# brdav/refign

Measured on AMD Instinct MI355X. Metric: image-pairs/s (align+seg fwd+bwd, 1080x1920), higher is better.
Workload: dtype bf16

## Files before the change

### include/refign_hip.h

```cpp
#ifndef REFIGN_HIP_H
#define REFIGN_HIP_H

#ifdef __cplusplus
extern "C" {
#endif

#define RFN_OK 0
#define RFN_EINVAL (-1)
#define RFN_ELAUNCH (-2)
#define RFN_ENOTSUP (-3)
#define RFN_ENONDET (-4)

#define RFN_ABI_VERSION 5

typedef void* rfn_stream_t;

int rfn_abi_version(void);
const char* rfn_last_error(void);

int rfn_set_deterministic(int on);
int rfn_get_deterministic(void);

int rfn_corr_fwd_f32(const float* in1, const float* in2, float* out, int B, int C, int iH, int iW,
                     int kH, int kW, int patchH, int patchW, int padH, int padW, int dilH, int dilW,
// ... 96 lines not shown

unsigned long rfn_sum_rows_workspace_bytes(long S, long n);
int rfn_sum_rows(const void* x, float* out, void* workspace, long S, long n, int x_dtype, int accumulate,
                 rfn_stream_t stream);
int rfn_linear_param_grads(const void* grad_y, float* grad_bias, void* workspace, long T, long N, int acc_bias,
                           const void* w_partials, float* grad_weight, int S, long NK, int acc_weight, int dtype,
                           rfn_stream_t stream);

int rfn_multi_cast_chunk_elems(void);
int rfn_multi_permute_chunk_elems(void);
int rfn_multi_permute_cast_f32(const void* table, int nchunks, rfn_stream_t stream);
int rfn_multi_cast_f32_bf16(const void* table, int nchunks, rfn_stream_t stream);
int rfn_multi_cast_f32_f16(const void* table, int nchunks, rfn_stream_t stream);
int rfn_multi_ema_f32(const void* table, int nchunks, float momentum, rfn_stream_t stream);
int rfn_multi_transpose_cast_f32_bf16(const void* table, int ntiles, rfn_stream_t stream);
int rfn_multi_transpose_cast_f32_f16(const void* table, int ntiles, rfn_stream_t stream);
int rfn_multi_transpose_tile(void);
int rfn_multi_adamw_f32(const void* table, int nchunks, const float* group_args, int ngroups, rfn_stream_t stream);
int rfn_amp_unscale_f32(float* grads, long n, const float* scale, float* found_inf, rfn_stream_t stream);
int rfn_multi_adamw_amp_f32(const void* table, int nchunks, const double* group_args, int ngroups, const float* found_inf,
                            const float* step, rfn_stream_t stream);
int rfn_amp_update_scale(float* scale, int* growth_tracker, const float* found_inf, float* step, float growth_factor,
                         float backoff_factor, int growth_interval, rfn_stream_t stream);

int rfn_upsample_concat_nhwc(const void* src0, const void* src1, const void* src2, const void* src3, const int* hs,
                             const int* ws, const int* cs, int nlev, void* out, int n, int H, int W, int dtype,
                             rfn_stream_t stream);
int rfn_upsample_concat_nhwc_bwd(const void* grad_out, void* grad0, void* grad1, void* grad2, void* grad3, const int* hs,
                                 const int* ws, const int* cs, int nlev, int n, int H, int W, int dtype,
                                 rfn_stream_t stream);

int rfn_patchify_tokens(const void* src, void* dst, int B, int H, int W, int C, int r, int dtype, int inverse,
                        rfn_stream_t stream);

int rfn_patchify_tokens_cmajor(const void* src, void* dst, int B, int H, int W, int C, int r, int dtype, int inverse,
                               rfn_stream_t stream);

int rfn_gemm_nt(const void* X, const void* W, const void* bias, const void* res, const float* rowscale,
                int rows_per_sample, int act, void* Y, long M, long N, long K, long ldx, long ldw, long ldy, int dtype,
                rfn_stream_t stream);
int rfn_conv2d_nhwc(const void* X, const void* W, const void* bias, const void* res, int act, void* Y, int B, int H,
                    int Wd, int C, int N, int KH, int KW, int stride, int pad, int dil, long ldw, long ldy, int dtype,
                    rfn_stream_t stream);
int rfn_gemm_tn(const void* G, const void* X, float* P, long T, long N, long K, long ldg, long ldx, int rows_per_slab,
                int accumulate, float* grad_bias, const float* rowscale, int rows_per_sample, int dtype,
                rfn_stream_t stream);
int rfn_gemm_tn_grouped(int count, const void* const* G, const void* const* X, float* const* P, float* const* grad_bias,
                        const float* const* rowscale, const long* T, const long* N, const long* K, const long* ldg,
                        const long* ldx, const int* rows_per_slab, const int* rows_per_sample, int dtype, rfn_stream_t stream);

int rfn_attn_pack(const void* src, long batch_stride, long row_stride, int B, int heads, int nrows, int nblk, void* rpack,
                  void* tpack, const void* src2, void* rpack2, void* tpack2, rfn_stream_t stream);
int rfn_attn_fwd(const void* Q, long q_batch_stride, long q_row_stride, const void* k_rpack, const void* v_tpack, void* O,
                 long o_batch_stride, long o_row_stride, float* lse2, int B, int heads, int Nq, int Nkv, int nkblk,
                 int nqpad, float scale, int kv_pack_heads, int dtype, rfn_stream_t stream);
int rfn_attn_bwd_dq(const void* Q, long q_batch_stride, long q_row_stride, const void* dO, const void* O,
                    long o_batch_stride, long o_row_stride, const void* k_rpack, const void* v_rpack, const void* k_tpack,
                    const float* lse2, float* delta, void* dQ, long dq_batch_stride, long dq_row_stride, int B, int heads,
                    int Nq, int Nkv, int nkblk, int nqpad, float scale, int kv_pack_heads, int dtype,
                    rfn_stream_t stream);
int rfn_attn_bwd_dkv(const void* K, const void* V, long kv_batch_stride, long kv_row_stride, const void* q_rpack,
                     const void* q_tpack, const void* do_rpack, const void* do_tpack, const float* lse2,
                     const float* delta, float* accT, void* dKV, int B, int heads, int Nq, int Nkv, int nqblk, int nqpad,
                     int nkpad, int blocks_per_chunk, float scale, int dtype, rfn_stream_t stream);

int rfn_attn32_fwd(const float* Q, long q_batch_stride, long q_row_stride, const float* KV, long kv_batch_stride,
                   long kv_row_stride, float* O, long o_batch_stride, long o_row_stride, float* lse2, int B, int heads,
                   int head_dim, int Nq, int Nkv, int nqpad, float scale, rfn_stream_t stream);
int rfn_attn32_bwd(const float* Q, long q_batch_stride, long q_row_stride, const float* KV, long kv_batch_stride,
                   long kv_row_stride, const float* dO, const float* O, long o_batch_stride, long o_row_stride,
                   const float* lse2, float* delta, float* dQ, long dq_batch_stride, long dq_row_stride, float* dKV,
                   long dkv_batch_stride, long dkv_row_stride, int B, int heads, int head_dim, int Nq, int Nkv, int nqpad,
                   int query_chunks, float scale, rfn_stream_t stream);

int rfn_split3_bf16(const float* x, long x_row_stride, void* out, long out_row_stride, long term_stride, long rows, int K,
                    int Kp, int order, rfn_stream_t stream);
int rfn_split3_cat_bf16(const float* const* parts, const long* strides, const int* channels, int nparts, void* out, int B, int H,
                        int W, int Cp, rfn_stream_t stream);

int rfn_ffn_fc1_dw_gelu_bf16(const void* x, const void* w1, const void* b1, const float* wdw_tap, const float* bdw, void* a,
                             int views, int H, int W, int C, int HID, rfn_stream_t stream);
int rfn_ffn_fc1_dw_gelu_f16(const void* x, const void* w1, const void* b1, const float* wdw_tap, const float* bdw, void* a,
                            int views, int H, int W, int C, int HID, rfn_stream_t stream);

int rfn_bn_stats_fwd(const void* x, double* sums, long T, int C, int dtype, rfn_stream_t stream);
int rfn_bn_apply_fwd(const void* x, const float* gamma, const float* beta, void* y, const double* sums, float* running_mean,
                     float* running_var, long T, int C, float eps, float momentum, int relu, int dtype, rfn_stream_t stream);
int rfn_bn_apply_fwd_ld(const void* x, const float* gamma, const float* beta, void* y, long ld_y, const double* sums,
                        float* running_mean, float* running_var, long T, int C, float eps, float momentum, int relu, int dtype,
                        rfn_stream_t stream);
int rfn_bn_stats_bwd(const void* x, const void* grad_y, const double* fwd_sums, const float* gamma, const float* beta,
                     float* bwd_sums, long T, int C, float eps, int relu, int dtype, rfn_stream_t stream);
int rfn_bn_apply_bwd(const void* x, const void* grad_y, const double* fwd_sums, const float* bwd_sums, const float* gamma,
                     const float* beta, void* grad_x, long T, int C, float eps, int relu, int dtype, rfn_stream_t stream);
int rfn_bn_train_fwd(const void* x, const float* gamma, const float* beta, void* y, double* sums, float* running_mean,
                     float* running_var, long T, int C, float eps, float momentum, int relu, int dtype,
                     rfn_stream_t stream);
int rfn_bn_train_bwd(const void* x, const void* grad_y, const double* fwd_sums, const float* gamma, const float* beta,
                     void* grad_x, float* bwd_sums, long T, int C, float eps, int relu, int dtype, rfn_stream_t stream);

int rfn_upsample_ce(const void* logits, const long* target, const float* weight, float* grad_lo, double* loss_sum, int B,
                    int C, int h, int w, int H, int W, int ignore_index, int dtype, int round16, rfn_stream_t stream);

int rfn_slide_argmax_confmat(const void* crop_logits, int dtype, int B, int C, int h, int w, const int* boxes, int nbox, int H,
                             int W, const long* target, int ignore_index, unsigned char* labels, long* confmat,
                             rfn_stream_t stream);

int rfn_gemm_nt_o32(const void* X, const void* W, const float* bias, const float* res, const float* rowscale,
                    int rows_per_sample, int act, float* Y, long M, long N, long K, long ldx, long ldw, long ldy,
                    rfn_stream_t stream);
int rfn_conv2d_nhwc_o32(const void* X, const void* W, const float* bias, int act, float* Y, int B, int H, int Wd, int C, int N,
                        int KH, int KW, int stride, int pad, int dil, long ldw, long ldy, int transposed,
                        rfn_stream_t stream);
int rfn_conv2d_nhwc_dgrad(const void* GY, const void* Wt, void* DX, int B, int H, int W, int C, int N, int KH, int KW,
                          int stride, int pad, int dil, long ldw, long ldy, int dtype, rfn_stream_t stream);
int rfn_conv2d_nhwc_wgrad(const void* GY, const void* X, float* P, float* grad_bias, int B, int H, int W, int C, int N, int KH,
                          int KW, int stride, int pad, int dil, long ldg, long Kpad, int rows_per_slab, int accumulate,
                          int dtype, rfn_stream_t stream);

int rfn_dacs_mix_jitter(const float* src, const float* trg, const long* gt_src, const long* pseudo_label,
                        const float* pseudo_weight, float* mixed_img, long* mixed_lbl, float* mixed_weight, double* mean_ws,
                        int B, int H, int W, const long* class_bits, const int* jitter_on, const int* order,
                        const float* factor, const float* hue, const float* mean3, const float* std3,
                        rfn_stream_t stream);
int rfn_dacs_blur(const float* x, float* tmp, float* y, int B, int C, int H, int W, int ksize_y, int ksize_x, const int* blur_on,
                  const double* sigma_y, const double* sigma_x, rfn_stream_t stream);

int rfn_crop_label_hist_u8(const void* label, int H, int W, const int* boxes, int K, int* hist, rfn_stream_t stream);
int rfn_crop_flip_norm_u8(const void* image, const void* label, int C, int H, int W, int top, int left, int h, int w, int flip,
                          const float* mean3, const float* std3, float* out_image, long* out_label, rfn_stream_t stream);

int rfn_resize_crop_flip_norm_u8(const void* image_hwc, int H, int W, int Hd, int Wd, const int* bounds_x, const int* coef_x, int kmax_x,
                                 const int* bounds_y, const int* coef_y, int kmax_y, int top, int left, int h, int w, int flip,
                                 const float* mean3, const float* std3, float* out_image, rfn_stream_t stream);
int rfn_resize_u8(const void* image_hwc, int H, int W, int Hd, int Wd, const int* bounds_x, const int* coef_x, int kmax_x,
                  const int* bounds_y, const int* coef_y, int kmax_y, void* out_chw, rfn_stream_t stream);
int rfn_resize_nearest_u8(const void* label, int H, int W, int Hd, int Wd, const int* ytab, const int* xtab, void* out,
                          rfn_stream_t stream);

int rfn_resize_filter_u8(const void* image_hwc, int H, int W, int Hd, int Wd, int filter, const int* bounds_x, const int* coef_x,
                         int kmax_x, const int* bounds_y, const int* coef_y, int kmax_y, void* out_chw, rfn_stream_t stream);
int rfn_resize_filter_crop_flip_norm_pad_u8(const void* image_hwc, int H, int W, int Hd, int Wd, int filter, const int* bounds_x,
                                            const int* coef_x, int kmax_x, const int* bounds_y, const int* coef_y, int kmax_y, int top,
                                            int left, int h, int w, int flip, const float* mean3, const float* std3, float* out_image,
                                            int Hf, int Wf, rfn_stream_t stream);

int rfn_sparse_epe_f32(const float* flow, const float* conf, const float* pts_src, const float* pts_trg, const int* offsets, int B,
                       int h, int w, double* rows, rfn_stream_t stream);

int rfn_gemm_nt_f8(const void* X8, const void* W8, const float* wscale, float x_scale, const void* bias, const void* res,
                   const float* rowscale, int rows_per_sample, int act, void* Y, int out_f8, float out_q, long M, long N,
                   long K, long ldx, long ldw, long ldy, rfn_stream_t stream);
int rfn_quant_rows_f8(const void* table, int nchunks, rfn_stream_t stream);
int rfn_quant_f8(const void* x_bf16, void* y8, long n, float q, rfn_stream_t stream);
int rfn_layernorm_fwd_f8(const void* x_bf16, const float* gamma, const float* beta, void* y8, long rows, int C, float eps,
                         float out_q, rfn_stream_t stream);
int rfn_dwconv3x3_gelu_nhwc_fwd_f8(const void* x8, const float* weight, const float* bias, void* y8, int B, int H, int W, int C,
                                   float x_scale, float out_q, rfn_stream_t stream);
int rfn_attn_pack_f8(const void* kv8, long batch_stride, long row_stride, int B, int heads, int Nkv, int nst, void* pack,
                     rfn_stream_t stream);
int rfn_attn_fwd_f8(const void* q8, long q_batch_stride, long q_row_stride, const void* pack, void* o8, long o_batch_stride,
                    long o_row_stride, int B, int heads, int Nq, int Nkv, int nst, float scale, float q_scale, float k_scale,
                    float v_scale, float out_q, rfn_stream_t stream);

unsigned long rfn_bn_stats_det_workspace_bytes(long T, int C);
int rfn_bn_stats_fwd_det(const void* x, double* sums, void* workspace, long T, int C, int dtype, rfn_stream_t stream);
// ... 77 lines not shown
```

### refign_amd/mfma.py

```python
import ctypes
import os

import torch

from . import _lib, determinism
from ._tensor import ptr
from ._tensor import DTYPE_CODE16 as _DT16

ENABLED = True

LIBRARY_CALLS = {}
_NOTE = True


def note_library(kind, *tensors):
    if not _NOTE or not tensors or not tensors[0].is_cuda:
        return
    key = (kind, str(tensors[0].dtype).replace("torch.", ""), tuple(tuple(t.shape) for t in tensors))
    n = LIBRARY_CALLS.get(key)
    if n is None and len(LIBRARY_CALLS) < 4096:
        if os.environ.get("RFN_LOG_LIBRARY", "0") == "1":
            print(f"[refign_amd] library fallback: {kind} {key[1]} {key[2]}", flush=True)
        LIBRARY_CALLS[key] = 1
    elif n is not None:
# ... 222 lines not shown
            X = arr(vp, [t[1].data_ptr() for t in grp])
            P = arr(vp, [t[2].data_ptr() for t in grp])
            Bv = arr(vp, [None if t[3] is None else t[3].data_ptr() for t in grp])
            R = arr(vp, [None if t[4] is None else t[4].data_ptr() for t in grp])
            T = arr(lg, [t[0].shape[0] for t in grp])
            N = arr(lg, [t[0].shape[1] for t in grp])
            K = arr(lg, [t[1].shape[1] for t in grp])
            ldg = arr(lg, [t[0].stride(0) for t in grp])
            ldx = arr(lg, [t[1].stride(0) for t in grp])
            rps = arr(it_, [t[6] for t in grp])
            rsa = arr(it_, [t[5] for t in grp])
            cast = lambda a_: ctypes.cast(a_, vp)
            _lib.call("rfn_gemm_tn_grouped", dev, n, cast(G), cast(X), cast(P), cast(Bv), cast(R), cast(T), cast(N), cast(K),
                      cast(ldg), cast(ldx), cast(rps), cast(rsa), _DT16[dt])


class deferred_wgrads:

    def __enter__(self):
        global _WGRAD_QUEUE
        self._outer = _WGRAD_QUEUE
        if GROUP_WGRADS and ENABLED and self._outer is None:
            _WGRAD_QUEUE = []
        return self

    def __exit__(self, *exc):
        global _WGRAD_QUEUE
        if self._outer is None and _WGRAD_QUEUE is not None:
            try:
                if exc[0] is None:
                    flush_wgrads()
            finally:
                _WGRAD_QUEUE = None
        return False


class _WgradMark(torch.autograd.Function):

    @staticmethod
    def forward(ctx, x):
        return x.view_as(x)

    @staticmethod
    def backward(ctx, g):
        flush_wgrads()
        return g


def wgrad_mark(x):
    return _WgradMark.apply(x) if (GROUP_WGRADS and torch.is_grad_enabled() and x.requires_grad) else x


_PACK_BLOCK = 4096


def _pack(src, batch_stride, row_stride, B, heads, nrows, nblk, want_r=True, want_t=True, src2=None):
    dev = src.device
    nbytes = B * heads * nblk * _PACK_BLOCK
    new = lambda want: torch.empty(nbytes, dtype=torch.uint8, device=dev) if want else None
    r, t = new(want_r), new(want_t)
    r2, t2 = (new(want_r), new(want_t)) if src2 is not None else (None, None)
    _lib.call("rfn_attn_pack", dev, ptr(src), batch_stride, row_stride, B, heads, nrows, nblk, ptr(r), ptr(t), ptr(src2),
              ptr(r2), ptr(t2))
    return (r, t), (r2, t2)


def _attn_ok(q, kv, heads):
    if not (ENABLED and q.is_cuda and q.dtype in _DT16 and kv.dtype == q.dtype and q.dim() == 3 and kv.dim() == 3):
        return False
    B, N, C = q.shape
    return (C == heads * 64 and kv.shape[0] == B and kv.shape[2] == 2 * C and q.is_contiguous() and kv.is_contiguous()
            and q.data_ptr() % 16 == 0 and kv.data_ptr() % 16 == 0)


def _dims(q, kv):
    B, N, C = q.shape
    Nkv = kv.shape[1]
    nkblk = -(-Nkv // 32)
    nkblk += nkblk & 1
    nqblk = -(-N // 32)
    return B, N, C, Nkv, nkblk, nqblk, nqblk * 32


def _fwd(q, kv, heads, scale, need_bwd):
    B, N, C, Nkv, nkblk, nqblk, nqpad = _dims(q, kv)
    dev = q.device
    (kvr, kvt), _ = _pack(kv, kv.stride(0), kv.stride(1), B, 2 * heads, Nkv, nkblk)
    voff = heads * nkblk * _PACK_BLOCK
    o = torch.empty_like(q)
    lse2 = torch.empty((B * heads, nqpad), dtype=torch.float32, device=dev)
    _lib.call("rfn_attn_fwd", dev, ptr(q), q.stride(0), q.stride(1), kvr.data_ptr(), kvt.data_ptr() + voff, ptr(o), o.stride(0),
              o.stride(1), ptr(lse2), B, heads, N, Nkv, nkblk, nqpad, float(scale), 2 * heads, _DT16[q.dtype])
    return o, lse2, (kvr, kvt)


def _chunk_blocks(nqblk, Nkv, BH):
    kblocks = -(-Nkv // 256)
    chunks = max(1, 128 // max(1, kblocks * BH))
    return max(4, -(-nqblk // chunks))


class _AttnFn(torch.autograd.Function):
    @staticmethod
    def forward(ctx, q, kv, heads, scale):
        need = q.requires_grad or kv.requires_grad
        o, lse2, packs = _fwd(q, kv, heads, scale, need)
        if need:
            ctx.save_for_backward(q, kv, o, lse2, *packs)
            ctx.heads, ctx.scale = heads, scale
        return o

    @staticmethod
    def backward(ctx, do):
        q, kv, o, lse2, kvr, kvt = ctx.saved_tensors
        heads, scale = ctx.heads, ctx.scale
        B, N, C, Nkv, nkblk, nqblk, nqpad = _dims(q, kv)
        dev = q.device
        if do.dtype != q.dtype:
            do = do.to(q.dtype)
        if not do.is_contiguous():
            do = do.contiguous()
        dt = _DT16[q.dtype]
        dq = torch.empty_like(q)
        delta = torch.empty_like(lse2)
        voff = heads * nkblk * _PACK_BLOCK
        _lib.call("rfn_attn_bwd_dq", dev, ptr(q), q.stride(0), q.stride(1), ptr(do), ptr(o), o.stride(0), o.stride(1),
                  kvr.data_ptr(), kvr.data_ptr() + voff, kvt.data_ptr(), ptr(lse2), ptr(delta), ptr(dq), dq.stride(0),
                  dq.stride(1), B, heads, N, Nkv, nkblk, nqpad, float(scale), 2 * heads, dt)
        (qr, qt), (gr, gt) = _pack(q, q.stride(0), q.stride(1), B, heads, N, nqblk, src2=do)
        nkpad = -(-Nkv // 32) * 32
        chunk = _chunk_blocks(nqblk, Nkv, B * heads)
        det = determinism.enabled()
        images = -(-nqblk // chunk) if det else 1
        accT = torch.empty(images * B * heads * 2 * 64 * nkpad, dtype=torch.float32, device=dev)
        dkv = torch.empty_like(kv)
        k_view, v_view = kv[:, :, :C], kv[:, :, C:]
        _lib.call("rfn_attn_bwd_dkv_det" if det else "rfn_attn_bwd_dkv", dev, ptr(k_view), ptr(v_view), kv.stride(0), kv.stride(1),
                  ptr(qr), ptr(qt), ptr(gr), ptr(gt), ptr(lse2), ptr(delta), ptr(accT), ptr(dkv), B, heads, N, Nkv, nqblk, nqpad,
                  nkpad, chunk, float(scale), dt)
        return dq, dkv, None, None


def attention(q, kv, heads, scale):
    if not _attn_ok(q, kv, heads):
        return None
    return _AttnFn.apply(q, kv, heads, scale)
```

### refign_amd/seg.py

```python
import math
import os
import random
from functools import partial, wraps
from typing import Callable, List, Optional, Union

import torch
import torch.nn as nn
import torch.nn.functional as F

from . import f8 as _f8
from . import linear as _linear
from . import determinism, mfma
from ._tensor import const_tensor
from ._tensor import DTYPE_CODE as _CE_DT
from .align import BaseHead
from .conv import Conv2d, patch_conv_tokens
from .layernorm import LayerNorm
from .layers import MLP, ConvBNReLU, DropPath
from .linear import Linear
from .upcat import upsample_concat
from .upsample import interpolate_bilinear

_MIT = {
    'mit_b0': ([32, 64, 160, 256], [2, 2, 2, 2]),
# ... 9 lines not shown

_GRAD_READY_CB = None


class _GradMark(torch.autograd.Function):

    @staticmethod
    def forward(ctx, x, tag):
        ctx.tag = tag
        return x.view_as(x)

    @staticmethod
    def backward(ctx, g):
        cb = _GRAD_READY_CB
        if cb is not None:
            cb(ctx.tag)
        return g, None


def grad_mark(x, tag):
    return _GradMark.apply(x, tag) if (torch.is_grad_enabled() and x.requires_grad) else x


class DWConv(nn.Module):

    def __init__(self, dim=768):
        super().__init__()
        self.dwconv = nn.Conv2d(dim, dim, 3, 1, 1, bias=True, groups=dim)

    def forward(self, x, H, W):
        B, N, C = x.shape
        if x.is_cuda and C % 8 == 0:
            from .dwconv import dwconv3x3_tokens
            return dwconv3x3_tokens(x, self.dwconv.weight, self.dwconv.bias, H, W)
        y = self.dwconv(x.transpose(1, 2).reshape(B, C, H, W))
        return y.flatten(2).transpose(1, 2)


class Mlp(nn.Module):

    def __init__(self, in_features, hidden_features=None, out_features=None, act_layer=nn.GELU, drop=0.):
        super().__init__()
        out_features = out_features or in_features
        hidden_features = hidden_features or in_features
        self.fc1 = Linear(in_features, hidden_features)
        self.dwconv = DWConv(hidden_features)
        self.act = act_layer()
        self.fc2 = Linear(hidden_features, out_features)
        self.drop = nn.Dropout(drop)

    def forward(self, x, H, W, res=None, rowscale=None):
        if x.is_cuda and not torch.is_grad_enabled() and x.dtype in (torch.bfloat16, torch.float16) and type(self.act) is nn.GELU \
                and self.act.approximate == 'none' and self.drop.p == 0. and type(self.fc1) is Linear and not _f8.active():
            from .dwconv import ffn_fc1_dw_gelu
            a = ffn_fc1_dw_gelu(x, self.fc1, self.dwconv.dwconv, H, W)
            if a is not None:
                return self.fc2(a, res=res, rowscale=rowscale) if res is not None else self.fc2(a)
        x = self.fc1(x)
        if x.is_cuda and x.shape[-1] % 8 == 0 and type(self.act) is nn.GELU and self.act.approximate == 'none':
            from .dwconv import dwconv3x3_gelu_tokens
            dw = self.dwconv.dwconv
            if torch.is_grad_enabled() and x.requires_grad and self.drop.p == 0. and x.dtype in (torch.bfloat16, torch.float16) \
                    and os.environ.get("RFN_FUSED_GELU_BWD", "1") == "1":
                a, z = dwconv3x3_gelu_tokens(x, dw.weight, dw.bias, H, W, with_z=True)
                if res is not None:
                    return self.fc2(a, res=res, rowscale=rowscale, z=z)
                return self.fc2(a, z=z)
            x = self.drop(dwconv3x3_gelu_tokens(x, dw.weight, dw.bias, H, W))
        else:
            x = self.drop(self.act(self.dwconv(x, H, W)))
        if res is not None and self.drop.p == 0.:
            return self.fc2(x, res=res, rowscale=rowscale)
        y = self.drop(self.fc2(x))
        return y if res is None else _residual(res, y, rowscale)


_SDPA_BACKEND = None
_FUSED_UPCAT = True


def _fused_upcat_here():
    return _FUSED_UPCAT
_SR_AS_LINEAR = True


class Attention(nn.Module):

    def __init__(self, dim, num_heads=8, qkv_bias=False, qk_scale=None, attn_drop=0., proj_drop=0., sr_ratio=1):
        super().__init__()
        assert dim % num_heads == 0, f'dim {dim} should be divided by num_heads {num_heads}.'
        self.dim, self.num_heads = dim, num_heads
        self.scale = qk_scale or (dim // num_heads) ** -0.5
        self.q = Linear(dim, dim, bias=qkv_bias)
        self.kv = Linear(dim, dim * 2, bias=qkv_bias)
        self.attn_drop = nn.Dropout(attn_drop)
        self.proj = Linear(dim, dim)
        self.proj_drop = nn.Dropout(proj_drop)
        self.sr_ratio = sr_ratio
        if sr_ratio > 1:
            self.sr = Conv2d(dim, dim, kernel_size=sr_ratio, stride=sr_ratio)
            self.norm = LayerNorm(dim)

    def forward(self, x, H, W, res=None, rowscale=None, x_kv=None):
        B, N, C = x.shape
        h, d = self.num_heads, C // self.num_heads
        q = self.q(x)
        if x_kv is not None:
            x = x_kv
        if self.sr_ratio > 1:
            r = patch_conv_tokens(x, H, W, self.sr) if _SR_AS_LINEAR else None
            if r is None:
                r = self.sr(x.transpose(1, 2).reshape(B, C, H, W)).flatten(2).transpose(1, 2)
            x = self.norm(r)
        kv = self.kv(x)
        p = self.attn_drop.p if self.training else 0.0
        o = mfma.attention(q, kv, h, self.scale) if (d == 64 and p == 0.0 and _SDPA_BACKEND is None) else None
        if o is None and q.is_cuda and q.dtype == torch.float32 and p == 0.0 and _SDPA_BACKEND is None:
            from . import split32
            if split32.usable(q, kv) and d in (32, 64):
                o = split32.attention(q, kv, h, self.scale)
        if o is None:
            mfma.note_library("sdpa", q, kv)
            q = q.view(B, N, h, d).transpose(1, 2)
            k, v = kv.view(B, -1, 2, h, d).permute(2, 0, 3, 1, 4).unbind(0)
            if _SDPA_BACKEND is None:
                o = F.scaled_dot_product_attention(q, k, v, dropout_p=p, scale=self.scale)
            else:
                with torch.nn.attention.sdpa_kernel([_SDPA_BACKEND]):
                    o = F.scaled_dot_product_attention(q, k, v, dropout_p=p, scale=self.scale)
            o = o.transpose(1, 2).reshape(B, N, C)
        if res is not None and self.proj_drop.p == 0.:
            return self.proj(o, res=res, rowscale=rowscale)
        y = self.proj_drop(self.proj(o))
        return y if res is None else _residual(res, y, rowscale)


def _residual(res, y, rowscale):
    if rowscale is None:
        return res + y
    return torch.addcmul(res, y, rowscale.to(y.dtype).view((-1,) + (1,) * (y.dim() - 1)))


_LN_PASS = True


_LN_FAN2 = True


def _norm_pass(norm, x, fan=1):
    if _LN_PASS and x.is_cuda and torch.is_grad_enabled() and x.requires_grad and type(norm) is LayerNorm and x.shape[-1] % 8 == 0 \
            and x.shape[-1] <= 1024 and x.dtype in (torch.float32, torch.bfloat16, torch.float16) and len(norm.normalized_shape) == 1:
        from .layernorm import layer_norm_pass, layer_norm_pass2
        if fan == 2 and _LN_FAN2:
            n, nb, xa = layer_norm_pass2(x, norm.weight, norm.bias, norm.eps)
            return (n, nb), xa
        n, xa = layer_norm_pass(x, norm.weight, norm.bias, norm.eps)
        return ((n, None), xa) if fan == 2 else (n, xa)
    n = norm(x)
    return ((n, None), x) if fan == 2 else (n, x)


class Block(nn.Module):

    def __init__(self, dim, num_heads, mlp_ratio=4., qkv_bias=False, qk_scale=None, drop=0., attn_drop=0.,
                 drop_path=0., act_layer=nn.GELU, norm_layer=LayerNorm, sr_ratio=1):
        super().__init__()
        self.norm1 = norm_layer(dim)
        self.attn = Attention(dim, num_heads=num_heads, qkv_bias=qkv_bias, qk_scale=qk_scale, attn_drop=attn_drop,
                              proj_drop=drop, sr_ratio=sr_ratio)
        self.drop_path = DropPath(drop_path) if drop_path > 0. else nn.Identity()
        self.norm2 = norm_layer(dim)
        self.mlp = Mlp(in_features=dim, hidden_features=int(dim * mlp_ratio), act_layer=act_layer, drop=drop)

    def forward(self, x, H, W, masks=None, masks32=None):
        if x.is_cuda and not torch.is_grad_enabled() and (masks is None) == (masks32 is None) and \
                (masks is not None or not (self.training and isinstance(self.drop_path, DropPath)
                                           and self.drop_path.drop_prob > 0.)):
            if _f8.active() and _f8.block_supported(self, x):
                return _f8.block_forward(self, x, H, W, masks32)
            x = self.attn(self.norm1(x), H, W, res=x, rowscale=None if masks32 is None else masks32[0])
            return self.mlp(self.norm2(x), H, W, res=x, rowscale=None if masks32 is None else masks32[1])
        x = mfma.wgrad_mark(x)
        if masks is not None:
            if x.is_cuda and masks32 is not None and _linear._FUSED_RESIDUAL:
                (n, nb), xa = _norm_pass(self.norm1, x, fan=2)
                x = self.attn(n, H, W, res=xa, rowscale=masks32[0], x_kv=nb)
                n, xa = _norm_pass(self.norm2, x)
                return self.mlp(n, H, W, res=xa, rowscale=masks32[1])
            x = torch.addcmul(x, self.attn(self.norm1(x), H, W), masks[0])
            return torch.addcmul(x, self.mlp(self.norm2(x), H, W), masks[1])
        dp = self.drop_path
        if x.is_cuda and _linear._FUSED_RESIDUAL and not (self.training and isinstance(dp, DropPath) and dp.drop_prob > 0.):
            (n, nb), xa = _norm_pass(self.norm1, x, fan=2)
            x = self.attn(n, H, W, res=xa, x_kv=nb)
            n, xa = _norm_pass(self.norm2, x)
            return self.mlp(n, H, W, res=xa)
        res = dp.residual if isinstance(dp, DropPath) else torch.add
        x = res(x, self.attn(self.norm1(x), H, W))
        return res(x, self.mlp(self.norm2(x), H, W))


class OverlapPatchEmbed(nn.Module):

    def __init__(self, img_size=224, patch_size=7, stride=4, in_chans=3, embed_dim=768):
        super().__init__()
        self.proj = Conv2d(in_chans, embed_dim, kernel_size=patch_size, stride=stride, padding=patch_size // 2)
        self.norm = LayerNorm(embed_dim)

    def forward(self, x):
        x = self.proj(x)
        H, W = x.shape[-2:]
        return self.norm(x.flatten(2).transpose(1, 2)), H, W

# ... 540 lines not shown
```

Measured before the change: 17.09.

## Fuse spatial-reduction conv, LayerNorm and KV projection into one packing kernel

Adds a HIP kernel that takes tokens, applies the strided spatial-reduction conv as an MFMA GEMM, runs LayerNorm in LDS, then computes the KV projection. It writes K and V straight into the packed layouts the attention kernel consumes. Attention uses this path when gradients are disabled, skipping the separate conv, norm, linear and pack launches and their intermediate tensors. The risk is that it only applies in no-grad inference and for four (C, r) shapes, and it adds LDS-heavy register pressure.

```diff
diff --git a/include/refign_hip.h b/include/refign_hip.h
--- a/include/refign_hip.h
+++ b/include/refign_hip.h
@@ -202,6 +202,10 @@
                              int views, int H, int W, int C, int HID, rfn_stream_t stream);
 int rfn_ffn_fc1_dw_gelu_f16(const void* x, const void* w1, const void* b1, const float* wdw_tap, const float* bdw, void* a,
                             int views, int H, int W, int C, int HID, rfn_stream_t stream);
+
+int rfn_kv_path(const void* x, const void* w_sr, const void* b_sr, const float* gamma, const float* beta, float eps,
+                const void* w_kv, const void* b_kv, void* k_rpack, void* v_tpack, void* kv_out, int B, int H, int W, int C,
+                int r, int nkblk, int blocks_per_wg, int dtype, rfn_stream_t stream);
 
 int rfn_bn_stats_fwd(const void* x, double* sums, long T, int C, int dtype, rfn_stream_t stream);
 int rfn_bn_apply_fwd(const void* x, const float* gamma, const float* beta, void* y, const double* sums, float* running_mean,
diff --git a/refign_amd/csrc/kvpath.hip b/refign_amd/csrc/kvpath.hip
--- /dev/null
+++ b/refign_amd/csrc/kvpath.hip
@@ -0,0 +1,397 @@
+#include "common.h"
+#include "mfma.h"
+
+namespace rfn {
+
+constexpr int kKvBlocks = 3;
+constexpr int kKvSmall = 128;
+constexpr int kKvPack = 4096;
+constexpr int kKvSPitch = 64 + 8;
+
+template <int C, int R, int NB> struct KvGeom {
+  static constexpr int ROWS = 32 * NB;
+  static constexpr int KSTEP = C <= 128 ? 128 : 64;
+  static constexpr int XP = KSTEP + 8, YP = C + 8;
+  static constexpr int YBYTES = ROWS * YP * 2;
+  static constexpr int XBYTES = R > 1 ? ROWS * XP * 2 : 0;
+  static constexpr int WSCR = 32 * ((R > 1 && KSTEP > 64 ? KSTEP : 64) + 8) * 2;
+  static constexpr int SBYTES = 4 * WSCR;
+  static constexpr int LDS = YBYTES + 2 * XBYTES + SBYTES;
+  static_assert(C % 64 == 0 && (R == 1 || (R * C) % KSTEP == 0), "a K-step never straddles a run of the gather");
+  static_assert(LDS <= 160 * 1024, "LDS");
+};
+
+template <int DT> __device__ __forceinline__ void kv_ld8(const uint16_t* p, float (&v)[8]) {
+  const u32x4 t = *(const u32x4*)p;
+  float a[4], b[4];
+  unpack4<DT>(u32x2{t[0], t[1]}, a);
+  unpack4<DT>(u32x2{t[2], t[3]}, b);
+#pragma unroll
+  for (int i = 0; i < 4; ++i) {
+    v[i] = a[i];
+    v[4 + i] = b[i];
+  }
+}
+
+template <int DT, int C, int R, int NB>
+__global__ __launch_bounds__(256) void kvpath_kernel(const uint16_t* __restrict__ X, const uint16_t* __restrict__ Wsr,
+                                                     const uint16_t* __restrict__ bsr, const float* __restrict__ gamma,
+                                                     const float* __restrict__ beta, float eps, const uint16_t* __restrict__ Wkv,
+                                                     const uint16_t* __restrict__ bkv, unsigned char* __restrict__ kr,
+                                                     unsigned char* __restrict__ vt, uint16_t* __restrict__ kvout, int B, int H,
+                                                     int W, int Wr, int Nkv, int nkblk) {
+  using E = Elem<DT>;
+  using vec8 = typename E::vec8;
+  using G = KvGeom<C, R, NB>;
+  constexpr int kKvBlocks = NB, kKvRows = G::ROWS;
+  constexpr int CB = C / 32, HEADS = C / 64, NCH = 2 * HEADS;
+  constexpr int YP = G::YP;
+  __shared__ __attribute__((aligned(16))) unsigned char smem[G::LDS];
+  uint16_t* yt = (uint16_t*)smem;
+  unsigned char* scr = smem + G::YBYTES + 2 * G::XBYTES;
+
+  const int t = threadIdx.x, lane = t & 63, col = lane & 31, g = lane >> 5;
+  const int wave = __builtin_amdgcn_readfirstlane(t >> 6);
+  const int nblocks = B * nkblk, gb0 = blockIdx.x * kKvBlocks;
+  auto row_of = [&](int tr, int& b, int& blk, int& row) {
+    const int gb = gb0 + (tr >> 5);
+    b = gb / nkblk;
+    blk = gb - b * nkblk;
+    row = blk * 32 + (tr & 31);
+    return gb < nblocks && row < Nkv;
+  };
+
+  if constexpr (R > 1) {
+    constexpr int KSTEP = G::KSTEP, XP = G::XP, NKS = KSTEP / 16, K1 = R * R * C;
+    constexpr int PPR = KSTEP / 8, RPP = 256 / PPR, NI = kKvRows / RPP;
+    constexpr int NCW = CB >= 4 ? (CB + 3) / 4 : 1, NTW = CB >= 4 ? kKvBlocks : (kKvBlocks + 1) / 2;
+    static_assert(CB >= 4 || CB == 2, "wave map");
+    const int sub = t % PPR, rb = t / PPR;
+    unsigned xo[NI];
+#pragma unroll
+    for (int i = 0; i < NI; ++i) {
+      int b, blk, row;
+      const bool ok = row_of(rb + RPP * i, b, blk, row);
+      const int oy = row / Wr, ox = row - oy * Wr;
+      xo[i] = (ok ? (unsigned)(((b * H + oy * R) * W + ox * R) * C) : 0u) + sub * 8;
+    }
+    auto fetch_x = [&](int k0, u32x4(&rx)[NI]) {
+      const int ry = k0 / (R * C);
+      const unsigned off = (unsigned)(ry * W * C + (k0 - ry * R * C));
+#pragma unroll
+      for (int i = 0; i < NI; ++i) rx[i] = *(const u32x4*)(X + (xo[i] + off));
+    };
+    auto stash_x = [&](int buf, const u32x4(&rx)[NI]) {
+      unsigned char* xs = smem + G::YBYTES + buf * G::XBYTES + (rb * XP + sub * 8) * 2;
+#pragma unroll
+      for (int i = 0; i < NI; ++i) *(u32x4*)(xs + RPP * i * XP * 2) = rx[i];
+    };
+    int cbc[NCW], tbc[NTW];
+    bool cb_ok[NCW], tb_ok[NTW];
+#pragma unroll
+    for (int i = 0; i < NCW; ++i) {
+      const int cb = CB >= 4 ? wave + 4 * i : (wave & 1);
+      cb_ok[i] = cb < CB;
+      cbc[i] = min(cb, CB - 1);
+    }
+#pragma unroll
+    for (int j = 0; j < NTW; ++j) {
+      const int tb = CB >= 4 ? j : (wave >> 1) + 2 * j;
+      tb_ok[j] = tb < kKvBlocks;
+      tbc[j] = min(tb, kKvBlocks - 1);
+    }
+    constexpr int WP = KSTEP + 8, PPW = KSTEP / 8, RPI = 64 / PPW;
+    static_assert(32 / RPI == NKS, "instructions per block");
+    const int wr = lane / PPW, wp = lane % PPW;
+    const uint16_t* wrow[NCW];
+#pragma unroll
+    for (int i = 0; i < NCW; ++i) wrow[i] = Wsr + (long)(cbc[i] * 32 + wr) * K1 + wp * 8;
+    auto fetch_w = [&](int k0, vec8(&wf)[NCW][NKS]) {
+#pragma unroll
+      for (int i = 0; i < NCW; ++i)
+#pragma unroll
+        for (int q = 0; q < NKS; ++q) wf[i][q] = *(const vec8*)(wrow[i] + (long)q * RPI * K1 + k0);
+    };
+    unsigned char* wscr = scr + wave * G::WSCR;
+    auto to_frags = [&](const vec8(&raw)[NKS], vec8(&fr)[NKS]) {
+      asm volatile("" ::: "memory");
+#pragma unroll
+      for (int q = 0; q < NKS; ++q) *(vec8*)(wscr + ((q * RPI + wr) * WP + wp * 8) * 2) = raw[q];
+      asm volatile("" ::: "memory");
+#pragma unroll
+      for (int ks = 0; ks < NKS; ++ks) fr[ks] = *(const vec8*)(wscr + (col * WP + ks * 16 + 8 * g) * 2);
+      asm volatile("" ::: "memory");
+    };
+    f32x16 acc[NCW][NTW];
+#pragma unroll
+    for (int i = 0; i < NCW; ++i)
+#pragma unroll
+      for (int j = 0; j < NTW; ++j)
+#pragma unroll
+        for (int r = 0; r < 16; ++r) acc[i][j][r] = 0.f;
+    constexpr int nk = K1 / KSTEP;
+    auto kstep = [&](int s, vec8(&cur)[NCW][NKS], vec8(&far)[NCW][NKS], const u32x4(&rnext)[NI], u32x4(&rfar)[NI]) {
+      const bool more = s + 1 < nk;
+      if (s + 2 < nk) {
+        fetch_x((s + 2) * KSTEP, rfar);
+        fetch_w((s + 2) * KSTEP, far);
+      }
+      const unsigned char* xs = smem + G::YBYTES + (s & 1) * G::XBYTES;
+      auto xfrag = [&](int j, int ks) { return *(const vec8*)(xs + ((tbc[j] * 32 + col) * XP + ks * 16 + 8 * g) * 2); };
+      vec8 xall[NCW > 1 ? NKS : 1][NTW];
+      if constexpr (NCW > 1) {
+#pragma unroll
+        for (int ks = 0; ks < NKS; ++ks)
+#pragma unroll
+          for (int j = 0; j < NTW; ++j) xall[ks][j] = xfrag(j, ks);
+      }
+#pragma unroll
+      for (int i = 0; i < NCW; ++i) {
+        vec8 wfr[NKS];
+        to_frags(cur[i], wfr);
+#pragma unroll
+        for (int ks = 0; ks < NKS; ++ks)
+#pragma unroll
+          for (int j = 0; j < NTW; ++j) acc[i][j] = E::mma(wfr[ks], NCW > 1 ? xall[NCW > 1 ? ks : 0][j] : xfrag(j, ks), acc[i][j]);
+      }
+      if (more) stash_x((s + 1) & 1, rnext);
+      __syncthreads();
+    };
+    vec8 wf0[NCW][NKS], wf1[NCW][NKS], wf2[NCW][NKS];
+    u32x4 rxa[NI], rxb[NI];
+    static_assert(nk >= 2, "two steps in flight");
+    fetch_x(0, rxa);
+    fetch_w(0, wf0);
+    fetch_x(KSTEP, rxb);
+    fetch_w(KSTEP, wf1);
+    stash_x(0, rxa);
+    __syncthreads();
+#pragma unroll 1
+    for (int s = 0; s < nk; s += 6) {
+      kstep(s, wf0, wf2, rxb, rxa);
+      if (s + 1 < nk) kstep(s + 1, wf1, wf0, rxa, rxb);
+      if (s + 2 < nk) kstep(s + 2, wf2, wf1, rxb, rxa);
+      if (s + 3 < nk) kstep(s + 3, wf0, wf2, rxa, rxb);
+      if (s + 4 < nk) kstep(s + 4, wf1, wf0, rxb, rxa);
+      if (s + 5 < nk) kstep(s + 5, wf2, wf1, rxa, rxb);
+    }
+#pragma unroll
+    for (int i = 0; i < NCW; ++i)
+#pragma unroll
+      for (int j = 0; j < NTW; ++j) {
+        if (!(cb_ok[i] && tb_ok[j])) continue;
+        const int tok = tbc[j] * 32 + col;
+#pragma unroll
+        for (int q = 0; q < 4; ++q) {
+          const int n0 = cbc[i] * 32 + 8 * q + 4 * g;
+          float bf[4];
+          unpack4<DT>(*(const u32x2*)(bsr + n0), bf);
+          *(u32x2*)(yt + tok * YP + n0) = pack4<DT>(acc[i][j][4 * q] + bf[0], acc[i][j][4 * q + 1] + bf[1],
+                                                   acc[i][j][4 * q + 2] + bf[2], acc[i][j][4 * q + 3] + bf[3]);
+        }
+      }
+    __syncthreads();
+    {
+      constexpr int LPR = C <= 64 ? 8 : (C <= 128 ? 16 : (C <= 256 ? 32 : 64)), RPW = 64 / LPR;
+      const int ls = lane % LPR, grp = lane / LPR, c = ls * 8;
+      const bool act = c < C;
+      float gm[8], bt[8];
+#pragma unroll
+      for (int h = 0; h < 2; ++h) {
+        const f32x4 a = *(const f32x4*)(gamma + (act ? c : 0) + 4 * h), b = *(const f32x4*)(beta + (act ? c : 0) + 4 * h);
+#pragma unroll
+        for (int e = 0; e < 4; ++e) {
+          gm[4 * h + e] = a[e];
+          bt[4 * h + e] = b[e];
+        }
+      }
+      const float invC = 1.0f / (float)C;
+#pragma unroll 1
+      for (int it = 0; it < kKvRows / (4 * RPW); ++it) {
+        uint16_t* p = yt + ((it * 4 + wave) * RPW + grp) * YP + (act ? c : 0);
+        float v[8];
+        if (act) kv_ld8<DT>(p, v);
+        else {
+#pragma unroll
+          for (int i = 0; i < 8; ++i) v[i] = 0.0f;
+        }
+        float s = 0.0f;
+#pragma unroll
+        for (int i = 0; i < 8; ++i) s += v[i];
+#pragma unroll
+        for (int o = LPR / 2; o > 0; o >>= 1) s += __shfl_xor(s, o, 64);
+        const float mu = s * invC;
+        float q = 0.0f;
+#pragma unroll
+        for (int i = 0; i < 8; ++i) {
+          const float d = act ? v[i] - mu : 0.0f;
+          q = fmaf(d, d, q);
+        }
+#pragma unroll
+        for (int o = LPR / 2; o > 0; o >>= 1) q += __shfl_xor(q, o, 64);
+        const float rs = rsqrtf(q * invC + eps);
+        if (act) {
+          float o[8];
+#pragma unroll
+          for (int i = 0; i < 8; ++i) o[i] = fmaf((v[i] - mu) * rs, gm[i], bt[i]);
+          const u32x2 lo = pack4<DT>(o[0], o[1], o[2], o[3]), hi = pack4<DT>(o[4], o[5], o[6], o[7]);
+          *(u32x4*)p = u32x4{lo[0], lo[1], hi[0], hi[1]};
+        }
+      }
+    }
+    __syncthreads();
+  } else {
+    constexpr int PPR = C / 8;
+    for (int p = t; p < kKvRows * PPR; p += 256) {
+      const int tr = p / PPR, sub = p - tr * PPR;
+      int b, blk, row;
+      u32x4 v = {0u, 0u, 0u, 0u};
+      if (row_of(tr, b, blk, row)) v = *(const u32x4*)(X + ((long)b * Nkv + row) * C + sub * 8);
+      *(u32x4*)(yt + tr * YP + sub * 8) = v;
+    }
+    __syncthreads();
+  }
+
+  constexpr int NPASS = (NCH + 3) / 4;
+#pragma unroll 1
+  for (int pass = 0; pass < NPASS; ++pass) {
+    const int hc = pass * 4 + wave;
+    const bool hc_ok = hc < NCH;
+    const int hcc = min(hc, NCH - 1);
+    unsigned char* ws = scr + wave * G::WSCR;
+    const int wr = lane >> 3, wp = lane & 7;
+    const uint16_t* w2row = Wkv + (long)(hcc * 64 + wr) * C + wp * 8;
+    auto fetch_w2 = [&](int k0, vec8(&wf)[2][4]) {
+#pragma unroll
+      for (int a = 0; a < 2; ++a)
+#pragma unroll
+        for (int q = 0; q < 4; ++q) wf[a][q] = *(const vec8*)(w2row + (long)(a * 32 + q * 8) * C + k0);
+    };
+    auto to_frags2 = [&](const vec8(&raw)[4], vec8(&fr)[4]) {
+      asm volatile("" ::: "memory");
+#pragma unroll
+      for (int q = 0; q < 4; ++q) *(vec8*)(ws + ((q * 8 + wr) * kKvSPitch + wp * 8) * 2) = raw[q];
+      asm volatile("" ::: "memory");
+#pragma unroll
+      for (int ks = 0; ks < 4; ++ks) fr[ks] = *(const vec8*)(ws + (col * kKvSPitch + ks * 16 + 8 * g) * 2);
+      asm volatile("" ::: "memory");
+    };
+    f32x16 acc2[2][kKvBlocks];
+#pragma unroll
+    for (int a = 0; a < 2; ++a)
+#pragma unroll
+      for (int j = 0; j < kKvBlocks; ++j)
+#pragma unroll
+        for (int r = 0; r < 16; ++r) acc2[a][j][r] = 0.f;
+    auto kstep2 = [&](int s, vec8(&cur)[2][4], vec8(&far)[2][4]) {
+      if (s + 2 < HEADS) fetch_w2((s + 2) * 64, far);
+      vec8 yf[4][kKvBlocks];
+#pragma unroll
+      for (int ks = 0; ks < 4; ++ks)
+#pragma unroll
+        for (int j = 0; j < kKvBlocks; ++j) yf[ks][j] = *(const vec8*)(yt + (j * 32 + col) * YP + s * 64 + ks * 16 + 8 * g);
+#pragma unroll
+      for (int a = 0; a < 2; ++a) {
+        vec8 wfr[4];
+        to_frags2(cur[a], wfr);
+#pragma unroll
+        for (int ks = 0; ks < 4; ++ks)
+#pragma unroll
+          for (int j = 0; j < kKvBlocks; ++j) acc2[a][j] = E::mma(wfr[ks], yf[ks][j], acc2[a][j]);
+      }
+    };
+    vec8 v0[2][4], v1[2][4], v2[2][4];
+    fetch_w2(0, v0);
+    if (HEADS > 1) fetch_w2(64, v1);
+#pragma unroll 1
+    for (int s = 0; s < HEADS; s += 3) {
+      kstep2(s, v0, v2);
+      if (s + 1 < HEADS) kstep2(s + 1, v1, v0);
+      if (s + 2 < HEADS) kstep2(s + 2, v2, v1);
+    }
+    const bool is_k = hc < HEADS;
+#pragma unroll
+    for (int j = 0; j < kKvBlocks; ++j) {
+      int b, blk, row;
+      const bool valid = row_of(j * 32 + col, b, blk, row);
+      const bool live = hc_ok && gb0 + j < nblocks;
+      const long pblk = ((long)(b * NCH + hcc) * nkblk + blk) * kKvPack;
+#pragma unroll
+      for (int a = 0; a < 2; ++a)
+#pragma unroll
+        for (int pr = 0; pr < 2; ++pr) {
+          float ba[4], bb[4];
+          const uint16_t* bp = bkv + hcc * 64 + a * 32 + 16 * pr + 4 * g;
+          unpack4<DT>(*(const u32x2*)bp, ba);
+          unpack4<DT>(*(const u32x2*)(bp + 8), bb);
+          const u32x2 pa = pack4<DT>(acc2[a][j][8 * pr] + ba[0], acc2[a][j][8 * pr + 1] + ba[1], acc2[a][j][8 * pr + 2] + ba[2],
+                                     acc2[a][j][8 * pr + 3] + ba[3]);
+          const u32x2 pb = pack4<DT>(acc2[a][j][8 * pr + 4] + bb[0], acc2[a][j][8 * pr + 5] + bb[1], acc2[a][j][8 * pr + 6] + bb[2],
+                                     acc2[a][j][8 * pr + 7] + bb[3]);
+          auto r0 = __builtin_amdgcn_permlane32_swap(pa[0], pb[0], false, false);
+          auto r1 = __builtin_amdgcn_permlane32_swap(pa[1], pb[1], false, false);
+          const u32x4 o = valid ? u32x4{r0[0], r1[0], r0[1], r1[1]} : u32x4{0u, 0u, 0u, 0u};
+          const int dc = a * 4 + 2 * pr + g;
+          if (live && is_k) *(u32x4*)(kr + pblk + (dc * 32 + col) * 16) = o;
+          if (live && valid && kvout != nullptr) *(u32x4*)(kvout + ((long)b * Nkv + row) * (2 * C) + hcc * 64 + dc * 8) = o;
+          *(u32x4*)(ws + (col * kKvSPitch + dc * 8) * 2) = o;
+        }
+      __syncthreads();
+      if (live && !is_k) {
+        const uint16_t* sc = (const uint16_t*)ws + lane;
+#pragma unroll
+        for (int rq = 0; rq < 8; ++rq) {
+          const unsigned h0 = sc[(4 * rq) * kKvSPitch], h1 = sc[(4 * rq + 1) * kKvSPitch], h2 = sc[(4 * rq + 2) * kKvSPitch],
+                         h3 = sc[(4 * rq + 3) * kKvSPitch];
+          *(u32x2*)(vt + pblk + (rq * 64 + lane) * 8) = u32x2{h0 | (h1 << 16), h2 | (h3 << 16)};
+        }
+      }
+      __syncthreads();
+    }
+  }
+}
+
+template <int DT, int C, int R, int NB>
+static int kvpath_launch(const void* x, const void* w_sr, const void* b_sr, const float* gamma, const float* beta, float eps,
+                         const void* w_kv, const void* b_kv, void* k_rpack, void* v_tpack, void* kv_out, int B, int H, int W, int Nkv,
+                         int nkblk, hipStream_t st) {
+  const int tiles = cdiv((long)B * nkblk, NB);
+  hipLaunchKernelGGL((kvpath_kernel<DT, C, R, NB>), dim3(tiles), dim3(256), 0, st, (const uint16_t*)x, (const uint16_t*)w_sr,
+                     (const uint16_t*)b_sr, gamma, beta, eps, (const uint16_t*)w_kv, (const uint16_t*)b_kv, (unsigned char*)k_rpack,
+                     (unsigned char*)v_tpack, (uint16_t*)kv_out, B, H, W, R > 1 ? W / R : 1, Nkv, nkblk);
+  return check_launch("kvpath_kernel");
+}
+
+}
+
+extern "C" int rfn_kv_path(const void* x, const void* w_sr, const void* b_sr, const float* gamma, const float* beta, float eps,
+                           const void* w_kv, const void* b_kv, void* k_rpack, void* v_tpack, void* kv_out, int B, int H, int W, int C,
+                           int r, int nkblk, int blocks_per_wg, int dtype, rfn_stream_t stream) {
+  using namespace rfn;
+  RFN_REQUIRE(x && w_kv && b_kv && k_rpack && v_tpack, "rfn_kv_path: null pointer");
+  RFN_REQUIRE(r == 1 || (w_sr && b_sr && gamma && beta), "rfn_kv_path: r = %d needs the spatial-reduction and LayerNorm parameters", r);
+  RFN_REQUIRE(B > 0 && H >= r && W >= r && r >= 1, "rfn_kv_path: B=%d H=%d W=%d r=%d", B, H, W, r);
+  RFN_REQUIRE((long)B * H * W * C < (1L << 31), "rfn_kv_path: B*H*W*C = %ld (32-bit element offsets)", (long)B * H * W * C);
+  const int Nkv = (H / r) * (W / r);
+  RFN_REQUIRE(nkblk % 2 == 0 && (long)nkblk * 32 >= Nkv && (long)B * nkblk < (1L << 24),
+              "rfn_kv_path: nkblk=%d (even, >= ceil(%d / 32))", nkblk, Nkv);
+  hipStream_t st = (hipStream_t)stream;
+  RFN_REQUIRE(blocks_per_wg == 0 || blocks_per_wg == 1 || blocks_per_wg == kKvBlocks, "rfn_kv_path: blocks_per_wg=%d (0, 1 or %d)",
+              blocks_per_wg, kKvBlocks);
+  const bool small = blocks_per_wg ? blocks_per_wg == 1 : cdiv((long)B * nkblk, kKvBlocks) < kKvSmall;
+  return dt16(dtype, "rfn_kv_path", [&](auto dtc) {
+    constexpr int DT = decltype(dtc)::value;
+#define RFN_KV(CC, RR)                                                                                                   \
+  if (C == CC && r == RR)                                                                                                \
+    return small ? kvpath_launch<DT, CC, RR, 1>(x, w_sr, b_sr, gamma, beta, eps, w_kv, b_kv, k_rpack, v_tpack, kv_out, B, H, W, Nkv, \
+                                                nkblk, st)                                                               \
+                 : kvpath_launch<DT, CC, RR, kKvBlocks>(x, w_sr, b_sr, gamma, beta, eps, w_kv, b_kv, k_rpack, v_tpack, kv_out, B, H, \
+                                                        W, Nkv, nkblk, st)
+    RFN_KV(64, 8);
+    RFN_KV(128, 4);
+    RFN_KV(320, 2);
+    RFN_KV(512, 1);
+#undef RFN_KV
+    return fail(RFN_EINVAL, "rfn_kv_path: (C, r) = (%d, %d): built for (64, 8), (128, 4), (320, 2), (512, 1)", C, r);
+  });
+}
diff --git a/refign_amd/mfma.py b/refign_amd/mfma.py
--- a/refign_amd/mfma.py
+++ b/refign_amd/mfma.py
@@ -328,16 +328,82 @@
     return B, N, C, Nkv, nkblk, nqblk, nqblk * 32
 
 
+def _nkblk(Nkv):
+    nkblk = -(-Nkv // 32)
+    return nkblk + (nkblk & 1)
+
+
+def _fwd_packed(q, kvr, kvt, heads, scale, Nkv, nkblk):
+    B, N, C = q.shape
+    nqpad = -(-N // 32) * 32
+    voff = heads * nkblk * _PACK_BLOCK
+    o = torch.empty_like(q)
+    lse2 = torch.empty((B * heads, nqpad), dtype=torch.float32, device=q.device)
+    _lib.call("rfn_attn_fwd", q.device, ptr(q), q.stride(0), q.stride(1), kvr.data_ptr(), kvt.data_ptr() + voff, ptr(o), o.stride(0),
+              o.stride(1), ptr(lse2), B, heads, N, Nkv, nkblk, nqpad, float(scale), 2 * heads, _DT16[q.dtype])
+    return o, lse2
+
+
 def _fwd(q, kv, heads, scale, need_bwd):
     B, N, C, Nkv, nkblk, nqblk, nqpad = _dims(q, kv)
-    dev = q.device
     (kvr, kvt), _ = _pack(kv, kv.stride(0), kv.stride(1), B, 2 * heads, Nkv, nkblk)
-    voff = heads * nkblk * _PACK_BLOCK
-    o = torch.empty_like(q)
-    lse2 = torch.empty((B * heads, nqpad), dtype=torch.float32, device=dev)
-    _lib.call("rfn_attn_fwd", dev, ptr(q), q.stride(0), q.stride(1), kvr.data_ptr(), kvt.data_ptr() + voff, ptr(o), o.stride(0),
-              o.stride(1), ptr(lse2), B, heads, N, Nkv, nkblk, nqpad, float(scale), 2 * heads, _DT16[q.dtype])
+    o, lse2 = _fwd_packed(q, kvr, kvt, heads, scale, Nkv, nkblk)
     return o, lse2, (kvr, kvt)
+
+
+KV_PATH_SHAPES = ((64, 8), (128, 4), (320, 2), (512, 1))
+
+
+def kv_packs(x, H, W, sr, norm, kv, want_kv=False, blocks_per_wg=0):
+    if not (ENABLED and x.is_cuda and x.dtype in _DT16 and x.dim() == 3 and x.is_contiguous() and x.data_ptr() % 16 == 0
+            and not torch.is_grad_enabled()):
+        return None
+    from .params import as_dtype, compute_dtype, derived
+    B, N, C = x.shape
+    cd = x.dtype
+    if compute_dtype(x) != cd or N != H * W or x.numel() >= 2 ** 31 or kv.bias is None or kv.weight.shape != (2 * C, C):
+        return None
+    if sr is None:
+        r, Nkv = 1, N
+        w_sr = b_sr = gamma = beta = None
+        eps = 0.0
+    else:
+        r = sr.kernel_size[0]
+        if not (sr.kernel_size == (r, r) and sr.stride == (r, r) and sr.padding == (0, 0) and sr.dilation == (1, 1)
+                and sr.groups == 1 and sr.bias is not None and sr.weight.shape[:2] == (C, C) and H >= r and W >= r
+                and tuple(norm.normalized_shape) == (C,) and norm.weight is not None and norm.bias is not None):
+            return None
+        Nkv = (H // r) * (W // r)
+    if (C, r) not in KV_PATH_SHAPES:
+        return None
+    if sr is not None:
+        w_sr = derived(sr.weight, (cd, "patch_linear"), lambda t: t.to(cd).permute(0, 2, 3, 1).contiguous(),
+                       lambda t: t.permute(0, 2, 3, 1))
+        b_sr = as_dtype(sr.bias, cd)
+        gamma, beta = as_dtype(norm.weight, torch.float32).detach(), as_dtype(norm.bias, torch.float32).detach()
+        eps = float(norm.eps)
+        if not (gamma.is_contiguous() and beta.is_contiguous()):
+            return None
+    w_kv, b_kv = as_dtype(kv.weight, cd), as_dtype(kv.bias, cd)
+    if not (w_kv.is_contiguous() and b_kv.is_contiguous()):
+        return None
+    heads, nkblk = C // 64, _nkblk(Nkv)
+    nbytes = B * 2 * heads * nkblk * _PACK_BLOCK
+    packs = torch.empty(2 * nbytes, dtype=torch.uint8, device=x.device)
+    kvr, kvt = packs[:nbytes], packs[nbytes:]
+    kv_out = torch.empty((B, Nkv, 2 * C), dtype=cd, device=x.device) if want_kv else None
+    _lib.call("rfn_kv_path", x.device, ptr(x), ptr(w_sr), ptr(b_sr), ptr(gamma), ptr(beta), eps, ptr(w_kv), ptr(b_kv), ptr(kvr),
+              ptr(kvt), ptr(kv_out), B, H if sr is not None else N, W if sr is not None else 1, C, r, nkblk,
+              int(blocks_per_wg), _DT16[cd])
+    return kvr, kvt, Nkv, nkblk, kv_out
+
+
+def attention_packed(q, packs, heads, scale):
+    if not (ENABLED and q.is_cuda and q.dtype in _DT16 and q.dim() == 3 and q.shape[2] == heads * 64 and q.is_contiguous()
+            and q.data_ptr() % 16 == 0 and not torch.is_grad_enabled()):
+        return None
+    kvr, kvt, Nkv, nkblk, _ = packs
+    return _fwd_packed(q, kvr, kvt, heads, scale, Nkv, nkblk)[0]
 
 
 def _chunk_blocks(nqblk, Nkv, BH):
diff --git a/refign_amd/seg.py b/refign_amd/seg.py
--- a/refign_amd/seg.py
+++ b/refign_amd/seg.py
@@ -115,6 +115,7 @@
 def _fused_upcat_here():
     return _FUSED_UPCAT
 _SR_AS_LINEAR = True
+_KV_FUSED = True
 
 
 class Attention(nn.Module):
@@ -140,13 +141,21 @@
         q = self.q(x)
         if x_kv is not None:
             x = x_kv
+        p = self.attn_drop.p if self.training else 0.0
+        if _KV_FUSED and not torch.is_grad_enabled() and x.is_cuda and d == 64 and p == 0.0 and _SDPA_BACKEND is None \
+                and q.dtype == x.dtype and type(self.kv) is Linear and not _f8.active() \
+                and (self.sr_ratio == 1 or (_SR_AS_LINEAR and type(self.norm) is LayerNorm)):
+            packs = mfma.kv_packs(x, H, W, self.sr if self.sr_ratio > 1 else None, self.norm if self.sr_ratio > 1 else None,
+                                  self.kv)
+            o = mfma.attention_packed(q, packs, h, self.scale) if packs is not None else None
+            if o is not None:
+                return self._project(o, res, rowscale)
         if self.sr_ratio > 1:
             r = patch_conv_tokens(x, H, W, self.sr) if _SR_AS_LINEAR else None
             if r is None:
                 r = self.sr(x.transpose(1, 2).reshape(B, C, H, W)).flatten(2).transpose(1, 2)
             x = self.norm(r)
         kv = self.kv(x)
-        p = self.attn_drop.p if self.training else 0.0
         o = mfma.attention(q, kv, h, self.scale) if (d == 64 and p == 0.0 and _SDPA_BACKEND is None) else None
         if o is None and q.is_cuda and q.dtype == torch.float32 and p == 0.0 and _SDPA_BACKEND is None:
             from . import split32
@@ -162,6 +171,9 @@
                 with torch.nn.attention.sdpa_kernel([_SDPA_BACKEND]):
                     o = F.scaled_dot_product_attention(q, k, v, dropout_p=p, scale=self.scale)
             o = o.transpose(1, 2).reshape(B, N, C)
+        return self._project(o, res, rowscale)
+
+    def _project(self, o, res, rowscale):
         if res is not None and self.proj_drop.p == 0.:
             return self.proj(o, res=res, rowscale=rowscale)
         y = self.proj_drop(self.proj(o))
```

After: 17.33 (median of 6 runs). 1.4% higher.
